# Antymon/ppo_cpp

Hardware: NVIDIA B200
Metric: ppo_env_steps_per_sec (higher is better)
Workload: dtype f32

## Files before the change

### ppo_cpp_b200/csrc/kernels_rollout.cuh

```cuda
#pragma once
#include <cooperative_groups.h>

#include "kernels_misc.cuh"
#include "kernels_mlp2.cuh"

namespace ppo {

struct RolloutArgs {
    NetDims d;
    const float* params;
    int n, T, tpc;
    uint64_t seed;
    uint32_t env_id0;
    uint32_t* step_ctr;
    SynthEnv env;
    NormStats st;
    float* ret;
    float norm_gamma, clip_obs, clip_rew, eps;
    int norm_obs, norm_reward, upd_obs, upd_ret;
    double* partial;
    float *cur_obs, *cur_dones, *last_values;
    float *obs_store, *act_store, *val_store, *nlp_store, *dones_store, *rew_store, *urew_store, *ret_store;
    float gamma, lam;
    unsigned *bar_ctr, *bar_gen;
    int n_global;
    PeerMailbox mbox;
    unsigned* mbox_seq;
    size_t off_obs, off_act, off_val, off_nlp, off_ret;
    size_t row_off;
    unsigned* done_seq;
    float* h_actions;
    size_t h_act_stride;
    const float *h_obs, *h_rew, *h_done;
    unsigned* h_act_flag;
    const unsigned* h_obs_flag;
    unsigned* host_err;
    int h_sentinel;
    uint2* h_act_ll;
    const uint2* h_ans_ll;
    long long* prof;
};

#define R_PROF()                                                                              \
    do {                                                                                      \
        if (a.prof && blockIdx.x == 0 && tid == 0 && t == 1 && prof_i < 32) a.prof[prof_i++] = clock64(); \
    } while (0)

constexpr int R_TM = 32, R_NTH = 256;
constexpr int R_SOLO_CHUNK = 32;
__host__ __device__ inline size_t rollout_solo_noise_bytes(int D) { return (size_t)2 * 2 * R_SOLO_CHUNK * 4 * ((D + 3) / 4) * sizeof(float) + 16; }
constexpr unsigned PPO_HOST_ENV_ABORT = 0xffffffffu;
constexpr unsigned PPO_OBS_SENTINEL = 0xffc0ffeeu;

__device__ __forceinline__ float* rslab(const RolloutArgs& a, int r, size_t off, int width, float* local) {
    return a.mbox.world > 1 ? reinterpret_cast<float*>(a.mbox.base[r] + off) + a.row_off * width : local;
}

struct RLayout {
    FLayout f;
    int obs, state, raw, ret, dn, tenv, res, rew, done, lastv, z2, mean, var, inv, misc, csum, total_bytes;
    __host__ __device__ void init(const NetDims& d, int tpc) {
        f.init(d, R_TM, false);
        int o = f.total;
        auto take = [&](int n) { int r = o; o += (n + 3) & ~3; return r; };
        obs = take(tpc * d.O * R_TM);
        state = take(tpc * d.O * R_TM);
        raw = take(tpc * d.O * R_TM);
        ret = take(tpc * R_TM); dn = take(tpc * R_TM); tenv = take(tpc * R_TM); res = take(tpc * R_TM);
        rew = take(tpc * R_TM); done = take(tpc * R_TM); lastv = take(tpc * R_TM);
        z2 = take(d.A * R_TM);
        mean = take(d.O + 1); var = take(d.O + 1); inv = take(d.O + 1); misc = take(8);
        o = (o + 1) & ~1;
        csum = o;
        o += 2 * (2 * (d.O + 1) + 2);
        total_bytes = o * 4;
    }
};

template <int O, int H1, int H2, int A, int TM>
__device__ __forceinline__ void solo_forward(const float* __restrict__ sW, const NetDims& d, const float* __restrict__ OBS, float* H1p, float* H1v,
                                             float* H2p, float* H2v, float* MU, float* Vs, int lane) {
#pragma unroll
    for (int i = 0; i < (2 * H1 + 31) / 32; ++i) {
        const int o = lane + 32 * i;
        if (o < 2 * H1) {
            const bool vt = o >= H1;
            const int n = vt ? o - H1 : o;
            const float* w = sW + d.off[vt ? T_VF_FC0_W : T_PI_FC0_W] + n;
            float acc = 0.f;
#pragma unroll
            for (int k = 0; k < O; ++k) acc = fmaf(w[k * H1], OBS[k * TM], acc);
            (vt ? H1v : H1p)[n * TM] = tanhf(acc + sW[d.off[vt ? T_VF_FC0_B : T_PI_FC0_B] + n]);
        }
    }
    __syncwarp();
#pragma unroll
    for (int i = 0; i < (2 * H2 + 31) / 32; ++i) {
        const int o = lane + 32 * i;
        if (o < 2 * H2) {
            const bool vt = o >= H2;
            const int n = vt ? o - H2 : o;
            const float* w = sW + d.off[vt ? T_VF_FC1_W : T_PI_FC1_W] + n;
            const float* hin = vt ? H1v : H1p;
            float acc = 0.f;
#pragma unroll
            for (int k = 0; k < H1; ++k) acc = fmaf(w[k * H2], hin[k * TM], acc);
            (vt ? H2v : H2p)[n * TM] = tanhf(acc + sW[d.off[vt ? T_VF_FC1_B : T_PI_FC1_B] + n]);
        }
    }
    __syncwarp();
    static_assert(A + 1 <= 32, "one lane per head output");
    if (lane < A + 1) {
        const bool vh = lane == A;
        const int N = vh ? 1 : A, n = vh ? 0 : lane;
        const float* w = sW + d.off[vh ? T_VF_W : T_PI_W] + n;
        const float* hin = vh ? H2v : H2p;
        float acc = 0.f;
#pragma unroll
        for (int k = 0; k < H2; ++k) acc = fmaf(w[k * N], hin[k * TM], acc);
        if (vh) Vs[0] = acc + sW[d.off[T_VF_B]];
        else MU[n * TM] = acc + sW[d.off[T_PI_B] + n];
    }
    __syncwarp();
}

__global__ void __launch_bounds__(R_NTH) rollout_persistent_kernel(const RolloutArgs a) {
    extern __shared__ __align__(16) float smem[];
    const NetDims& d = a.d;
    constexpr int TM = R_TM, NTH = R_NTH;
    const int O = d.O, A = d.A, D = d.O;
    RLayout L;
    L.init(d, a.tpc);
    float* sW = smem + L.f.w;
    float* Ac = smem + L.f.ac;
    float* MU = smem + L.f.mu;
    float* Vs = smem + L.f.vs;
    float* OBS = smem + L.obs;
    float* S = smem + L.state;
    float* RAW = smem + L.raw;
    float* RET = smem + L.ret;
    float* DN = smem + L.dn;
    uint32_t* TENV = reinterpret_cast<uint32_t*>(smem + L.tenv);
    uint32_t* RES = reinterpret_cast<uint32_t*>(smem + L.res);
    float* REW = smem + L.rew;
    float* DONE = smem + L.done;
    float* LASTV = smem + L.lastv;
    float* Z2 = smem + L.z2;
    float* s_mean = smem + L.mean;
    float* s_var = smem + L.var;
    float* s_inv = smem + L.inv;
    double* csum = reinterpret_cast<double*>(smem + L.csum);
    double* s_cnt = csum + 2 * (D + 1);

    const int tid = threadIdx.x, lane = tid & 31, warp = tid >> 5;
    constexpr int HALF = NTH / 2;
    const int tw = tid / HALF;
    const Sub half{tid % HALF, HALF};
    float* H1 = smem + L.f.h1[tw];
    float* H2 = smem + L.f.h2[tw];
    const int ntiles = (a.n + TM - 1) / TM;
    const int tile0 = blockIdx.x * a.tpc;
    const int my_tiles = max(0, min(a.tpc, ntiles - tile0));
    const int nblk = (D + 3) >> 2;
    const uint32_t step0 = *a.step_ctr;
    const bool merge = a.upd_obs || a.upd_ret;
    GridBarrier bar{a.bar_ctr, gridDim.x, *a.bar_gen};
    const int world = a.mbox.world;
    const bool host_env = a.h_actions != nullptr;
    __shared__ int s_abort;
    if (tid == 0) s_abort = 0;
    const unsigned seq0 = world > 1 ? *a.mbox_seq : 0u;
    const unsigned dseq0 = world > 1 ? *a.done_seq : 0u;

    stage_weights<NTH>(sW, a.params, d.P);
    if (tid < D) {
        s_mean[tid] = a.st.obs_mean[tid];
        s_var[tid] = a.st.obs_var[tid];
    } else if (tid == D) {
        s_mean[D] = *a.st.ret_mean;
        s_var[D] = *a.st.ret_var;
        s_cnt[0] = *a.st.obs_count;
        s_cnt[1] = *a.st.ret_count;
    }
    for (int tl = 0; tl < my_tiles; ++tl) {
        const int r0 = (tile0 + tl) * TM, nv = min(TM, a.n - r0);
        for (int e = tid; e < TM * D; e += NTH) {
            const int m = e / D, k = e - m * D;
            const bool ok = m < nv;
            OBS[(tl * O + k) * TM + m] = ok ? a.cur_obs[(size_t)(r0 + m) * O + k] : 0.f;
            S[(tl * TM + m) * D + k] = ok ? a.env.state[(size_t)(r0 + m) * D + k] : 0.f;
        }
        if (tid < TM) {
            const bool ok = tid < nv;
            RET[tl * TM + tid] = ok ? a.ret[r0 + tid] : 0.f;
            DN[tl * TM + tid] = ok ? a.cur_dones[r0 + tid] : 0.f;
            TENV[tl * TM + tid] = ok ? a.env.t_env[r0 + tid] : 0u;
            RES[tl * TM + tid] = ok ? a.env.resets[r0 + tid] : 0u;
        }
    }
    if (a.h_actions != nullptr && a.h_sentinel) {
        for (int tl = 0; tl < my_tiles; ++tl) {
            const int r0 = (tile0 + tl) * TM, nv = min(TM, a.n - r0);
            unsigned* dst = reinterpret_cast<unsigned*>(const_cast<float*>(a.h_obs) + (size_t)r0 * D);
            for (int i = tid; i < ((nv * D + 7) >> 3); i += NTH) dst[8 * i] = PPO_OBS_SENTINEL;
        }
    }
    cp_async_wait_all();
    bar.sync();

    const float* logstd = sW + d.off[T_LOGSTD];
    const uint2 ekey = make_uint2((uint32_t)a.env.seed, (uint32_t)(a.env.seed >> 32));

    int prof_i = 0;
    const bool solo_env = a.n == 1 && gridDim.x == 1 && world == 1;
    if (solo_env) {
        constexpr int CH = R_SOLO_CHUNK;
        const int NB = 4 * nblk;
        float* NZ = smem + ((L.total_bytes + 15) / 16) * 4;
        const uint32_t gid = a.env.env_id0;
        const uint32_t te0 = TENV[0];
        auto draw_chunk = [&](int c) {
            float* dst = NZ + (size_t)(c & 1) * 2 * CH * NB;
            const int per_kind = CH * nblk, total = host_env ? per_kind : 2 * per_kind;
            for (int e = tid - 32; e < total; e += NTH - 32) {
                const int kind = e / per_kind, r = e - kind * per_kind, s = r / nblk, blk = r - s * nblk, t = c * CH + s;
                if (t >= a.T) continue;
                float x4[4];
                if (kind == 0) normal4(a.seed, a.env_id0, step0 + (uint32_t)t, (uint32_t)blk, PPO_TAG_ACTION, x4);
                else normal4(a.env.seed, gid, te0 + (uint32_t)t, (uint32_t)blk, PPO_TAG_ENVNOISE, x4);
                float* o = dst + ((size_t)kind * CH + s) * NB + blk * 4;
                o[0] = x4[0]; o[1] = x4[1]; o[2] = x4[2]; o[3] = x4[3];
            }
        };
        if (warp > 0) draw_chunk(0);
        __syncthreads();
        float sl_c = 0.f;
        for (int j = 0; j < A; ++j) sl_c = __fadd_rn(sl_c, logstd[j]);
        const int nH1 = d.H1, nH2 = d.H2;
        const float *W0p = sW + d.off[T_PI_FC0_W], *W0v = sW + d.off[T_VF_FC0_W], *B0p = sW + d.off[T_PI_FC0_B], *B0v = sW + d.off[T_VF_FC0_B];
        const float *W1p = sW + d.off[T_PI_FC1_W], *W1v = sW + d.off[T_VF_FC1_W], *B1p = sW + d.off[T_PI_FC1_B], *B1v = sW + d.off[T_VF_FC1_B];
        const float *WHp = sW + d.off[T_PI_W], *WHv = sW + d.off[T_VF_W];
        float *H1p = smem + L.f.h1[0], *H1v = smem + L.f.h1[1], *H2p = smem + L.f.h2[0], *H2v = smem + L.f.h2[1];
        float sd_l[2];
        sd_l[0] = lane < A ? expf(logstd[lane]) : 1.f;
        sd_l[1] = lane + 32 < A ? expf(logstd[lane + 32]) : 1.f;
        for (int c = 0; c * CH < a.T; ++c) {
            if (warp > 0) {
                draw_chunk(c + 1);
            } else {
                const float* na = NZ + (size_t)(c & 1) * 2 * CH * NB;
                const float* ne = na + (size_t)CH * NB;
                for (int s = 0; s < CH && c * CH + s < a.T; ++s) {
                    const int t = c * CH + s;
                    R_PROF();
                    for (int k = lane; k < O; k += 32) a.obs_store[(size_t)t * O + k] = OBS[k * TM];
                    if (O == 18 && A == 18 && nH1 == 4 && nH2 == 5) {
                        solo_forward<18, 4, 5, 18, TM>(sW, d, OBS, H1p, H1v, H2p, H2v, MU, Vs, lane);
                    } else if (O == 18 && A == 18 && nH1 == 64 && nH2 == 64) {
                        solo_forward<18, 64, 64, 18, TM>(sW, d, OBS, H1p, H1v, H2p, H2v, MU, Vs, lane);
                    } else {
                    for (int o = lane; o < 2 * nH1; o += 32) {
                        const bool vt = o >= nH1;
                        const int n = vt ? o - nH1 : o;
                        const float* w = (vt ? W0v : W0p) + n;
                        float acc = 0.f;
#pragma unroll 6
                        for (int k = 0; k < O; ++k) acc = fmaf(w[k * nH1], OBS[k * TM], acc);
                        (vt ? H1v : H1p)[n * TM] = tanhf(acc + (vt ? B0v : B0p)[n]);
                    }
                    __syncwarp();
                    for (int o = lane; o < 2 * nH2; o += 32) {
                        const bool vt = o >= nH2;
                        const int n = vt ? o - nH2 : o;
                        const float* w = (vt ? W1v : W1p) + n;
                        const float* hin = vt ? H1v : H1p;
                        float acc = 0.f;
#pragma unroll 4
                        for (int k = 0; k < nH1; ++k) acc = fmaf(w[k * nH2], hin[k * TM], acc);
                        (vt ? H2v : H2p)[n * TM] = tanhf(acc + (vt ? B1v : B1p)[n]);
                    }
                    __syncwarp();
                    for (int o = lane; o < A + 1; o += 32) {
                        const bool vh = o == A;
                        const int N = vh ? 1 : A, n = vh ? 0 : o;
                        const float* w = (vh ? WHv : WHp) + n;
                        const float* hin = vh ? H2v : H2p;
                        float acc = 0.f;
#pragma unroll 4
                        for (int k = 0; k < nH2; ++k) acc = fmaf(w[k * N], hin[k * TM], acc);
                        if (vh) Vs[0] = acc + sW[d.off[T_VF_B]];
                        else MU[n * TM] = acc + sW[d.off[T_PI_B] + n];
                    }
                    __syncwarp();
                    }
                    R_PROF();
                    for (int j = lane, jj = 0; j < A; j += 32, ++jj) {
                        const float sd = jj ? sd_l[1] : sd_l[0];
                        const float mu = MU[j * TM];
                        const float act = __fadd_rn(mu, __fmul_rn(sd, na[s * NB + j]));
                        const float z = __fdiv_rn(__fsub_rn(act, mu), sd);
                        Ac[j * (TM + 1)] = act;
                        Z2[j * TM] = __fmul_rn(z, z);
                        a.act_store[(size_t)t * A + j] = act;
                        if (host_env) {
                            if (a.h_act_ll) ll_store(a.h_act_ll + j, __float_as_uint(act), (unsigned)t + 1u);
                            else a.h_actions[(size_t)t * a.h_act_stride + j] = act;
                        }
                    }
                    __syncwarp();
                    if (lane == 0) {
                        float ss = 0.f;
                        for (int j = 0; j < A; ++j) ss = __fadd_rn(ss, Z2[j * TM]);
                        a.nlp_store[t] = __fadd_rn(__fadd_rn(__fmul_rn(0.5f, ss), __fmul_rn(PPO_HALF_LOG_2PI, (float)A)), sl_c);
                        a.val_store[t] = Vs[0];
                        a.dones_store[t] = DN[0];
                    }
                    R_PROF();
                    if (host_env && a.h_ans_ll) {
                        const unsigned want = (unsigned)t + 1u;
                        uint2 w = make_uint2(0u, want);
                        bool gone = false;
                        if (lane < D + 2) {
                            const unsigned long long t0 = globaltimer_ns();
                            unsigned spins = 0;
                            while (true) {
                                w = ll_load(a.h_ans_ll + lane);
                                if (w.y == want) break;
                                if (w.y == PPO_HOST_ENV_ABORT) { gone = true; break; }
                                if (((++spins) & 0xffu) == 0u && globaltimer_ns() - t0 > 120000000000ull) {
                                    *a.host_err = 1u;
                                    gone = true;
                                    break;
                                }
                            }
                        }
                        if (__any_sync(0xffffffffu, gone)) {
                            if (lane == 0) s_abort = 1;
                            break;
                        }
                        if (lane < D) RAW[lane] = __uint_as_float(w.x);
                        else if (lane == D) REW[0] = __uint_as_float(w.x);
                        else if (lane == D + 1) DONE[0] = __uint_as_float(w.x);
                        __syncwarp();
                        if (lane == 0) RET[0] = __fadd_rn(__fmul_rn(RET[0], a.norm_gamma), REW[0]);
                    } else if (host_env) {
                        __syncwarp();
                        unsigned v = 0u;
                        if (lane == 0) {
                            __threadfence_system();
                            st_release_sys(a.h_act_flag, (unsigned)t + 1u);
                            const unsigned long long t0 = globaltimer_ns();
                            unsigned spins = 0;
                            while ((v = *reinterpret_cast<const volatile unsigned*>(a.h_obs_flag)) != (unsigned)t + 1u && v != PPO_HOST_ENV_ABORT) {
                                if (((++spins) & 0xffu) == 0u && globaltimer_ns() - t0 > 120000000000ull) {
                                    *a.host_err = 1u;
                                    v = PPO_HOST_ENV_ABORT;
                                    break;
                                }
                            }
                            __threadfence_system();
                        }
                        v = __shfl_sync(0xffffffffu, v, 0);
                        if (v == PPO_HOST_ENV_ABORT) {
                            if (lane == 0) s_abort = 1;
                            break;
                        }
                        for (int k = lane; k < D; k += 32) RAW[k] = __ldcv(a.h_obs + k);
                        if (lane == 0) {
                            REW[0] = __ldcv(a.h_rew);
                            DONE[0] = __ldcv(a.h_done);
                        }
                        __syncwarp();
                        if (lane == 0) RET[0] = __fadd_rn(__fmul_rn(RET[0], a.norm_gamma), REW[0]);
                    } else {
                        const uint32_t te = te0 + (uint32_t)t;
                        const bool dn = ((te + 1u) % 334u) == 0u;
                        for (int k = lane; k < D; k += 32) {
                            const float sk = S[k];
                            float ac = Ac[k * (TM + 1)];
                            ac = ac < -1.f ? -1.f : (ac > 1.f ? 1.f : ac);
                            float sn = __fadd_rn(__fadd_rn(__fmul_rn(0.9f, sk), __fmul_rn(0.1f, ac)), __fmul_rn(0.01f, ne[s * NB + k]));
                            if (k == 0) REW[0] = __fsub_rn(sn, sk);
                            if (dn) {
                                const uint4 w = philox4x32_10(make_uint4(gid, RES[0], (uint32_t)(k >> 2), PPO_TAG_ENVRESET), ekey);
                                const uint32_t wv[4] = {w.x, w.y, w.z, w.w};
                                sn = __fmul_rn(0.1f, __fsub_rn(__fmul_rn(2.0f, u32_to_unit(wv[k & 3])), 1.0f));
                            }
                            S[k] = sn;
                            RAW[k] = sn;
                        }
                        __syncwarp();
                        if (lane == 0) {
                            DONE[0] = dn ? 1.f : 0.f;
                            TENV[0] = te + 1u;
                            if (dn) RES[0] += 1u;
                            RET[0] = __fadd_rn(__fmul_rn(RET[0], a.norm_gamma), REW[0]);
                        }
                    }
                    __syncwarp();
                    R_PROF();
                    if (merge && lane <= D) {
                        const int cidx = lane;
                        const bool is_ret = cidx == D;
                        const double x = is_ret ? (double)RET[0] : (double)RAW[cidx] - (double)s_mean[cidx];
                        double ps = 0.0, pq = 0.0;
                        ps += x;
                        pq += x * x;
                        if (is_ret ? a.upd_ret : a.upd_obs) {
                            const double rows = (double)a.n_global;
                            const double pv = is_ret ? 0.0 : (double)s_mean[cidx];
                            const double m1 = ps;
                            const double mean_d = pv + m1;
                            double var_d = pq - m1 * m1;
                            if (var_d < 0.0) var_d = 0.0;
                            float mm = s_mean[cidx], vv = s_var[cidx];
                            chan_merge(mm, vv, s_cnt[is_ret ? 1 : 0], (float)mean_d, (float)var_d, rows);
                            s_mean[cidx] = mm;
                            s_var[cidx] = vv;
                        }
                    }
                    __syncwarp();
                    if (merge && lane == 0) {
                        if (a.upd_obs) s_cnt[0] = (double)a.n_global + s_cnt[0];
                        if (a.upd_ret) s_cnt[1] = (double)a.n_global + s_cnt[1];
                    }
                    R_PROF();
                    if (lane <= D) s_inv[lane] = __fdiv_rn(1.0f, __fsqrt_rn(__fadd_rn(s_var[lane], a.eps)));
                    __syncwarp();
                    for (int k = lane; k < D; k += 32) {
                        float x = RAW[k];
                        if (a.norm_obs) {
                            x = __fmul_rn(__fsub_rn(x, s_mean[k]), s_inv[k]);
                            x = fminf(fmaxf(x, -a.clip_obs), a.clip_obs);
                        }
                        OBS[k * TM] = x;
                    }
                    if (lane == 0) {
                        const float raw = REW[0];
                        float r = raw;
                        if (a.norm_reward) {
                            r = __fmul_rn(raw, s_inv[D]);
                            r = fminf(fmaxf(r, -a.clip_rew), a.clip_rew);
                        }
                        const float dn2 = DONE[0];
                        RET[0] = __fmul_rn(RET[0], __fsub_rn(1.0f, dn2));
                        DN[0] = dn2;
                        a.rew_store[t] = r;
                        a.urew_store[t] = raw;
                    }
                    __syncwarp();
                    R_PROF();
                }
            }
            __syncthreads();
            if (s_abort) break;
        }
    } else
    for (int t = 0; t < a.T; ++t) {
        const uint32_t step = step0 + (uint32_t)t;
        R_PROF();
        double ps = 0.0, pq = 0.0;
        const float pivot = (tid < D) ? s_mean[tid] : 0.f;
        for (int pass = 0; pass < (host_env ? 2 : 1); ++pass) {
        if (pass == 1) {
            __syncthreads();
            if (a.h_sentinel) {
                if (tid == 0) {
                    __threadfence_system();
                    st_release_sys(a.h_act_flag + blockIdx.x, (unsigned)t + 1u);
                }
                int gone = 0;
                const unsigned long long t0 = globaltimer_ns();
                for (int tl = 0; tl < my_tiles && !gone; ++tl) {
                    const int r0 = (tile0 + tl) * TM, nv = min(TM, a.n - r0);
                    const unsigned* src = reinterpret_cast<const unsigned*>(a.h_obs + (size_t)r0 * D);
                    const int nsec = (nv * D + 7) >> 3;
                    for (int i = tid; i < nsec && !gone; i += NTH) {
                        unsigned spins = 0;
                        while (__ldcv(src + 8 * i) == PPO_OBS_SENTINEL) {
                            if (((++spins) & 0x3fu) == 0u) {
                                if (__ldcv(a.h_obs_flag) == PPO_HOST_ENV_ABORT) { gone = 1; break; }
                                if (globaltimer_ns() - t0 > 120000000000ull) {
                                    *a.host_err = 1u;
                                    gone = 1;
                                    break;
                                }
                            }
                        }
                    }
                }
                const int any_gone = __syncthreads_or(gone);
                if (tid == 0) s_abort = any_gone;
                __syncthreads();
                if (s_abort) break;
            } else {
            if (tid == 0) {
                __threadfence_system();
                st_release_sys(a.h_act_flag + blockIdx.x, (unsigned)t + 1u);
                const unsigned long long t0 = globaltimer_ns();
                unsigned v, spins = 0;
                while ((v = *reinterpret_cast<const volatile unsigned*>(a.h_obs_flag)) != (unsigned)t + 1u && v != PPO_HOST_ENV_ABORT) {
                    if (((++spins) & 0xffu) == 0u && globaltimer_ns() - t0 > 120000000000ull) {
                        *a.host_err = 1u;
                        v = PPO_HOST_ENV_ABORT;
                        break;
                    }
                }
                s_abort = (v == PPO_HOST_ENV_ABORT) ? 1 : 0;
                __threadfence_system();
            }
            __syncthreads();
            if (s_abort) break;
            }
        }
        for (int tl = 0; tl < my_tiles; ++tl) {
            const int r0 = (tile0 + tl) * TM, nv = min(TM, a.n - r0);
            float* Xs = OBS + tl * O * TM;
            if (pass == 0) {
            for (int r = 0; r < world; ++r) {
                float* dst = rslab(a, r, a.off_obs, O, a.obs_store) + ((size_t)t * a.n + r0) * O;
                for (int e = tid; e < nv * O; e += NTH) {
                    const int m = e / O, k = e - m * O;
                    dst[e] = Xs[k * TM + m];
                }
            }
            f_fwd<TM, true>(Xs, O, sW + d.off[tw ? T_VF_FC0_W : T_PI_FC0_W], sW + d.off[tw ? T_VF_FC0_B : T_PI_FC0_B], d.H1, H1, half);
            __syncthreads();
            f_fwd<TM, true>(H1, d.H1, sW + d.off[tw ? T_VF_FC1_W : T_PI_FC1_W], sW + d.off[tw ? T_VF_FC1_B : T_PI_FC1_B], d.H2, H2, half);
            __syncthreads();
            if (tw == 0) f_fwd<TM, false>(H2, d.H2, sW + d.off[T_PI_W], sW + d.off[T_PI_B], A, MU, half);
            else f_fwd<TM, false>(H2, d.H2, sW + d.off[T_VF_W], sW + d.off[T_VF_B], 1, Vs, half);
            __syncthreads();
            R_PROF();
            for (int e = tid; e < TM * nblk; e += NTH) {
                const int m = e % TM, blk = e / TM;
                if (m < nv) {
                    float e4[4];
                    normal4(a.seed, a.env_id0 + (uint32_t)(r0 + m), step, (uint32_t)blk, PPO_TAG_ACTION, e4);
#pragma unroll
                    for (int q = 0; q < 4; ++q) {
                        const int j = blk * 4 + q;
                        if (j < A) {
                            const float sd = expf(logstd[j]);
                            const float mu = MU[j * TM + m];
                            const float act = __fadd_rn(mu, __fmul_rn(sd, e4[q]));
                            const float z = __fdiv_rn(__fsub_rn(act, mu), sd);
                            Ac[j * (TM + 1) + m] = act;
                            Z2[j * TM + m] = __fmul_rn(z, z);
                        }
                    }
                }
            }
            __syncthreads();
            if (tid < nv) {
                const int m = tid, row = r0 + m;
                float ss = 0.f, sl = 0.f;
                for (int j = 0; j < A; ++j) {
                    ss = __fadd_rn(ss, Z2[j * TM + m]);
                    sl = __fadd_rn(sl, logstd[j]);
                }
                const float nl = __fadd_rn(__fadd_rn(__fmul_rn(0.5f, ss), __fmul_rn(PPO_HALF_LOG_2PI, (float)A)), sl);
                const size_t idx = (size_t)t * a.n + row;
                for (int r = 0; r < world; ++r) {
                    rslab(a, r, a.off_nlp, 1, a.nlp_store)[idx] = nl;
                    rslab(a, r, a.off_val, 1, a.val_store)[idx] = Vs[m];
                }
                a.dones_store[idx] = DN[tl * TM + m];
            }
            for (int r = 0; r < world; ++r) {
                float* dst = rslab(a, r, a.off_act, A, a.act_store) + ((size_t)t * a.n + r0) * A;
                for (int e = tid; e < nv * A; e += NTH) {
                    const int m = e / A, j = e - m * A;
                    dst[e] = Ac[j * (TM + 1) + m];
                }
            }
            R_PROF();
            }
            if (host_env) {
                if (pass == 0) {
                    float* dst = a.h_actions + (size_t)t * a.h_act_stride + (size_t)r0 * A;
                    const int ne = nv * A;
                    if ((reinterpret_cast<uintptr_t>(dst) & 15) == 0) {
                        for (int e4 = tid; e4 < (ne >> 2); e4 += NTH) {
                            float v[4];
#pragma unroll
                            for (int i = 0; i < 4; ++i) {
                                const int e = 4 * e4 + i, m = e / A, j = e - m * A;
                                v[i] = Ac[j * (TM + 1) + m];
                            }
                            *reinterpret_cast<float4*>(dst + 4 * e4) = make_float4(v[0], v[1], v[2], v[3]);
                        }
                        for (int e = (ne & ~3) + tid; e < ne; e += NTH) {
                            const int m = e / A, j = e - m * A;
                            dst[e] = Ac[j * (TM + 1) + m];
                        }
                    } else {
                        for (int e = tid; e < ne; e += NTH) {
                            const int m = e / A, j = e - m * A;
                            dst[e] = Ac[j * (TM + 1) + m];
                        }
                    }
                    __syncthreads();
                    continue;
                }
                for (int e = tid; e < nv * D; e += NTH) RAW[tl * TM * D + e] = __ldcv(a.h_obs + (size_t)r0 * D + e);
                if (tid < nv) {
                    REW[tl * TM + tid] = __ldcv(a.h_rew + r0 + tid);
                    DONE[tl * TM + tid] = __ldcv(a.h_done + r0 + tid);
                }
                __syncthreads();
                if (a.h_sentinel) {
                    unsigned* dst = reinterpret_cast<unsigned*>(const_cast<float*>(a.h_obs) + (size_t)r0 * D);
                    for (int i = tid; i < ((nv * D + 7) >> 3); i += NTH) dst[8 * i] = PPO_OBS_SENTINEL;
                }
                if (tid < nv) RET[tl * TM + tid] = __fadd_rn(__fmul_rn(RET[tl * TM + tid], a.norm_gamma), REW[tl * TM + tid]);
                __syncthreads();
            } else {
            for (int e = tid; e < TM * nblk; e += NTH) {
                const int m = e % TM, blk = e / TM;
                if (m < nv) {
                    const uint32_t gid = a.env.env_id0 + (uint32_t)(r0 + m);
                    const uint32_t te = TENV[tl * TM + m];
                    const bool dn = ((te + 1u) % 334u) == 0u;
                    float xi[4];
                    normal4(a.env.seed, gid, te, (uint32_t)blk, PPO_TAG_ENVNOISE, xi);
                    float* st = S + (tl * TM + m) * D;
                    float* rw = RAW + (tl * TM + m) * D;
                    uint4 w = make_uint4(0, 0, 0, 0);
                    if (dn) w = philox4x32_10(make_uint4(gid, RES[tl * TM + m], (uint32_t)blk, PPO_TAG_ENVRESET), ekey);
                    const uint32_t wv[4] = {w.x, w.y, w.z, w.w};
#pragma unroll
                    for (int q = 0; q < 4; ++q) {
                        const int k = blk * 4 + q;
                        if (k < D) {
                            const float sk = st[k];
                            float ac = Ac[k * (TM + 1) + m];
                            ac = ac < -1.f ? -1.f : (ac > 1.f ? 1.f : ac);
                            float sn = __fadd_rn(__fadd_rn(__fmul_rn(0.9f, sk), __fmul_rn(0.1f, ac)), __fmul_rn(0.01f, xi[q]));
                            if (k == 0) REW[tl * TM + m] = __fsub_rn(sn, sk);
                            if (dn) sn = __fmul_rn(0.1f, __fsub_rn(__fmul_rn(2.0f, u32_to_unit(wv[q])), 1.0f));
                            st[k] = sn;
                            rw[k] = sn;
                        }
                    }
                    if (blk == 0) DONE[tl * TM + m] = dn ? 1.f : 0.f;
                }
            }
            __syncthreads();
            if (tid < nv) {
                const int m = tid;
                TENV[tl * TM + m] += 1u;
                if (DONE[tl * TM + m] != 0.f) RES[tl * TM + m] += 1u;
                RET[tl * TM + m] = __fadd_rn(__fmul_rn(RET[tl * TM + m], a.norm_gamma), REW[tl * TM + m]);
            }
            __syncthreads();
            }
            R_PROF();
            if (merge) {
                if (tid < D) {
                    for (int m = 0; m < nv; ++m) {
                        const double x = (double)RAW[(tl * TM + m) * D + tid] - (double)pivot;
                        ps += x;
                        pq += x * x;
                    }
                } else if (tid == D) {
                    for (int m = 0; m < nv; ++m) {
                        const double r = (double)RET[tl * TM + m];
                        ps += r;
                        pq += r * r;
                    }
                }
            }
        }
        }
        if (s_abort) break;
        if (merge) {
            const bool solo = gridDim.x == 1 && world == 1;
            double* mine = a.partial + (size_t)(t & 1) * 2 * (D + 1) * gridDim.x + blockIdx.x;
            if (solo) {
                if (tid <= D) {
                    csum[tid] = ps;
                    csum[D + 1 + tid] = pq;
                }
            } else if (tid <= D) {
                mine[(size_t)tid * gridDim.x] = ps;
                mine[(size_t)(D + 1 + tid) * gridDim.x] = pq;
            }
            R_PROF();
            if (!solo) bar.sync();
            R_PROF();
            const double* all = a.partial + (size_t)(t & 1) * 2 * (D + 1) * gridDim.x;
            if (!solo && (world == 1 || blockIdx.x == 0)) {
                constexpr int CPW = 5;
                double acc[CPW];
#pragma unroll
                for (int i = 0; i < CPW; ++i) acc[i] = 0.0;
#pragma unroll 4
                for (int b0 = 0; b0 < (int)gridDim.x; b0 += 32) {
                    double x[CPW];
#pragma unroll
                    for (int i = 0; i < CPW; ++i) {
                        const int c = warp + (NTH / 32) * i;
                        x[i] = (c < 2 * (D + 1) && b0 + lane < (int)gridDim.x) ? __ldcg(all + (size_t)c * gridDim.x + b0 + lane) : 0.0;
                    }
#pragma unroll
                    for (int i = 0; i < CPW; ++i) acc[i] += x[i];
                }
#pragma unroll
                for (int i = 0; i < CPW; ++i) {
                    const int c = warp + (NTH / 32) * i;
                    const double v = warp_sum(acc[i]);
                    if (lane == 0 && c < 2 * (D + 1)) csum[c] = v;
                }
                for (int c = (NTH / 32) * CPW + warp; c < 2 * (D + 1); c += NTH / 32) {
                    double v = 0.0;
                    for (int b = lane; b < (int)gridDim.x; b += 32) v += __ldcg(all + (size_t)c * gridDim.x + b);
                    v = warp_sum(v);
                    if (lane == 0) csum[c] = v;
                }
            }
            __syncthreads();
            if (world > 1) {
                const unsigned seq = seq0 + (unsigned)t + 1u;
                if (blockIdx.x == 0 && tid < 2 * (D + 1)) {
                    const unsigned long long bits = (unsigned long long)__double_as_longlong(csum[tid]);
                    for (int dst = 0; dst < world; ++dst) {
                        uint2* sl = a.mbox.ll_slot(dst, seq, a.mbox.rank) + 2 * tid;
                        ll_store(sl, (unsigned)bits, seq);
                        ll_store(sl + 1, (unsigned)(bits >> 32), seq);
                    }
                }
                __syncthreads();
                if (tid < 2 * (D + 1)) {
                    double v = 0.0;
                    for (int s0 = 0; s0 < world; s0 += 4) {
                        unsigned long long w[4];
                        a.mbox.ll_wait4_pair(seq, (size_t)(2 * tid), s0, w);
#pragma unroll
                        for (int k = 0; k < 4; ++k)
                            if (s0 + k < world) v += __longlong_as_double((long long)w[k]);
                    }
                    csum[tid] = v;
                }
                __syncthreads();
            }
            R_PROF();
            if (tid <= D) {
                const int c = tid;
                const bool is_ret = c == D;
                if (is_ret ? a.upd_ret : a.upd_obs) {
                    const double rows = (double)a.n_global;
                    const double pv = is_ret ? 0.0 : (double)s_mean[c];
                    const double m1 = csum[c] / rows;
                    const double mean_d = pv + m1;
                    double var_d = csum[D + 1 + c] / rows - m1 * m1;
                    if (var_d < 0.0) var_d = 0.0;
                    float mm = s_mean[c], vv = s_var[c];
                    chan_merge(mm, vv, s_cnt[is_ret ? 1 : 0], (float)mean_d, (float)var_d, rows);
                    s_mean[c] = mm;
                    s_var[c] = vv;
                }
            }
            __syncthreads();
            if (tid == 0) {
                if (a.upd_obs) s_cnt[0] = (double)a.n_global + s_cnt[0];
                if (a.upd_ret) s_cnt[1] = (double)a.n_global + s_cnt[1];
            }
        }
        R_PROF();
        if (tid <= D) s_inv[tid] = __fdiv_rn(1.0f, __fsqrt_rn(__fadd_rn(s_var[tid], a.eps)));
        __syncthreads();
        for (int tl = 0; tl < my_tiles; ++tl) {
            const int r0 = (tile0 + tl) * TM, nv = min(TM, a.n - r0);
            for (int e = tid; e < TM * D; e += NTH) {
                const int m = e / D, k = e - m * D;
                float x = RAW[(tl * TM + m) * D + k];
                if (a.norm_obs) {
                    x = __fmul_rn(__fsub_rn(x, s_mean[k]), s_inv[k]);
                    x = fminf(fmaxf(x, -a.clip_obs), a.clip_obs);
                }
                OBS[(tl * O + k) * TM + m] = (m < nv) ? x : 0.f;
            }
            if (tid < nv) {
                const int m = tid;
                const float raw = REW[tl * TM + m];
                float r = raw;
                if (a.norm_reward) {
                    r = __fmul_rn(raw, s_inv[D]);
                    r = fminf(fmaxf(r, -a.clip_rew), a.clip_rew);
                }
                const float dn = DONE[tl * TM + m];
                RET[tl * TM + m] = __fmul_rn(RET[tl * TM + m], __fsub_rn(1.0f, dn));
                DN[tl * TM + m] = dn;
                const size_t idx = (size_t)t * a.n + r0 + m;
                a.rew_store[idx] = r;
                a.urew_store[idx] = raw;
            }
        }
        __syncthreads();
        R_PROF();
    }

    for (int tl = 0; tl < my_tiles; ++tl) {
        const int r0 = (tile0 + tl) * TM, nv = min(TM, a.n - r0);
        float* Xs = OBS + tl * O * TM;
        if (tw == 1) f_fwd<TM, true>(Xs, O, sW + d.off[T_VF_FC0_W], sW + d.off[T_VF_FC0_B], d.H1, H1, half);
        __syncthreads();
        if (tw == 1) f_fwd<TM, true>(H1, d.H1, sW + d.off[T_VF_FC1_W], sW + d.off[T_VF_FC1_B], d.H2, H2, half);
        __syncthreads();
        if (tw == 1) f_fwd<TM, false>(H2, d.H2, sW + d.off[T_VF_W], sW + d.off[T_VF_B], 1, Vs, half);
        __syncthreads();
        if (tid < nv) LASTV[tl * TM + tid] = Vs[tid];
        for (int e = tid; e < nv * D; e += NTH) {
            const int m = e / D, k = e - m * D;
            a.cur_obs[(size_t)r0 * O + e] = Xs[k * TM + m];
            a.env.state[(size_t)r0 * D + e] = S[(tl * TM + m) * D + k];
        }
        __syncthreads();
    }
    for (int e = tid; e < my_tiles * TM; e += NTH) {
        const int tl = e / TM, m = e - tl * TM;
        const int row = (tile0 + tl) * TM + m;
        if (row >= a.n) continue;
        a.ret[row] = RET[e];
        a.cur_dones[row] = DN[e];
        a.env.t_env[row] = TENV[e];
        a.env.resets[row] = RES[e];
        a.last_values[row] = LASTV[e];
        const float gl = __fmul_rn(a.gamma, a.lam);
        float last = 0.f, nextv = LASTV[e], nextnt = 1.0f - DN[e];
#pragma unroll 8
        for (int t = a.T - 1; t >= 0; --t) {
            const size_t idx = (size_t)t * a.n + row;
            const float v = a.val_store[idx];
            const float delta = __fsub_rn(__fadd_rn(a.rew_store[idx], __fmul_rn(a.gamma, __fmul_rn(nextv, nextnt))), v);
            last = __fadd_rn(delta, __fmul_rn(gl, __fmul_rn(nextnt, last)));
            const float rt = __fadd_rn(last, v);
            for (int r = 0; r < world; ++r) rslab(a, r, a.off_ret, 1, a.ret_store)[idx] = rt;
            nextv = v;
            nextnt = 1.0f - a.dones_store[idx];
        }
    }
    if (world > 1) {
        __syncthreads();
        if (tid == 0) __threadfence_system();
        bar.sync();
        if (blockIdx.x == 0 && tid == 0) {
            a.mbox.signal_all(PPO_MBOX_DONE_CHANNEL, dseq0 + 1u);
            a.mbox.wait_all(PPO_MBOX_DONE_CHANNEL, dseq0 + 1u);
            *a.done_seq = dseq0 + 1u;
        }
    }
    if (blockIdx.x == 0) {
        if (tid < D) {
            a.st.obs_mean[tid] = s_mean[tid];
            a.st.obs_var[tid] = s_var[tid];
        } else if (tid == D) {
            *a.st.ret_mean = s_mean[D];
            *a.st.ret_var = s_var[D];
            *a.st.obs_count = s_cnt[0];
            *a.st.ret_count = s_cnt[1];
            *a.step_ctr = step0 + (uint32_t)a.T;
            *a.bar_gen = bar.gen;
            if (world > 1 && merge) *a.mbox_seq = seq0 + (unsigned)a.T;
        }
    }
}

}
```

Before: 36.93 million.

## Precompute action and env noise on idle threads during head layer

During the final head forward pass, threads not used by the policy/value head matmuls now generate the Philox normal noise for actions, environment noise and reset randoms, and store them in new shared-memory buffers. The later action-sampling and env-step loops read the precomputed noise instead of calling the RNG. The aim is to hide RNG latency inside an otherwise underused phase, at the cost of extra shared memory (which can lower occupancy) and a dependency on the idle-thread index arithmetic being correct. The profiling step index also changes.

After: 37.14 million (median of 6 runs). No clear change (+0.5%).

```diff
diff --git a/ppo_cpp_b200/csrc/kernels_rollout.cuh b/ppo_cpp_b200/csrc/kernels_rollout.cuh
--- a/ppo_cpp_b200/csrc/kernels_rollout.cuh
+++ b/ppo_cpp_b200/csrc/kernels_rollout.cuh
@@ -43,7 +43,7 @@
 
 #define R_PROF()                                                                              \
     do {                                                                                      \
-        if (a.prof && blockIdx.x == 0 && tid == 0 && t == 1 && prof_i < 32) a.prof[prof_i++] = clock64(); \
+        if (a.prof && blockIdx.x == 0 && tid == 0 && t == 8 && prof_i < 32) a.prof[prof_i++] = clock64(); \
     } while (0)
 
 constexpr int R_TM = 32, R_NTH = 256;
@@ -58,7 +58,7 @@
 
 struct RLayout {
     FLayout f;
-    int obs, state, raw, ret, dn, tenv, res, rew, done, lastv, z2, mean, var, inv, misc, csum, total_bytes;
+    int obs, state, raw, ret, dn, tenv, res, rew, done, lastv, z2, nza, nze, nzr, mean, var, inv, misc, csum, total_bytes;
     __host__ __device__ void init(const NetDims& d, int tpc) {
         f.init(d, R_TM, false);
         int o = f.total;
@@ -69,6 +69,8 @@
         ret = take(tpc * R_TM); dn = take(tpc * R_TM); tenv = take(tpc * R_TM); res = take(tpc * R_TM);
         rew = take(tpc * R_TM); done = take(tpc * R_TM); lastv = take(tpc * R_TM);
         z2 = take(d.A * R_TM);
+        const int nz = ((d.O + 3) / 4) * R_TM * 4;
+        nza = take(nz); nze = take(nz); nzr = take(nz);
         mean = take(d.O + 1); var = take(d.O + 1); inv = take(d.O + 1); misc = take(8);
         o = (o + 1) & ~1;
         csum = o;
@@ -146,6 +148,9 @@
     float* DONE = smem + L.done;
     float* LASTV = smem + L.lastv;
     float* Z2 = smem + L.z2;
+    float4* NZA = reinterpret_cast<float4*>(smem + L.nza);
+    float4* NZE = reinterpret_cast<float4*>(smem + L.nze);
+    uint4* NZR = reinterpret_cast<uint4*>(smem + L.nzr);
     float* s_mean = smem + L.mean;
     float* s_var = smem + L.var;
     float* s_inv = smem + L.inv;
@@ -530,13 +535,33 @@
             __syncthreads();
             if (tw == 0) f_fwd<TM, false>(H2, d.H2, sW + d.off[T_PI_W], sW + d.off[T_PI_B], A, MU, half);
             else f_fwd<TM, false>(H2, d.H2, sW + d.off[T_VF_W], sW + d.off[T_VF_B], 1, Vs, half);
+            {
+                const int hp = ((TM / 4) * ((A + 3) >> 2) + 31) & ~31, hv = ((TM / 4) + 31) & ~31;
+                const int idle = tw == 0 ? half.l - hp : (HALF - hp) + half.l - hv, nidle = 2 * HALF - hp - hv;
+                const int per = TM * nblk;
+                if (half.l >= (tw == 0 ? hp : hv))
+                    for (int e = idle; e < (host_env ? per : 2 * per); e += nidle) {
+                        const int kind = e >= per, r = e - kind * per, blk = r / TM, m = r - blk * TM;
+                        if (m >= nv) continue;
+                        float x4[4];
+                        if (kind == 0) {
+                            normal4(a.seed, a.env_id0 + (uint32_t)(r0 + m), step, (uint32_t)blk, PPO_TAG_ACTION, x4);
+                            NZA[r] = make_float4(x4[0], x4[1], x4[2], x4[3]);
+                        } else {
+                            const uint32_t gid = a.env.env_id0 + (uint32_t)(r0 + m), te = TENV[tl * TM + m];
+                            normal4(a.env.seed, gid, te, (uint32_t)blk, PPO_TAG_ENVNOISE, x4);
+                            NZE[r] = make_float4(x4[0], x4[1], x4[2], x4[3]);
+                            if (((te + 1u) % 334u) == 0u) NZR[r] = philox4x32_10(make_uint4(gid, RES[tl * TM + m], (uint32_t)blk, PPO_TAG_ENVRESET), ekey);
+                        }
+                    }
+            }
             __syncthreads();
             R_PROF();
             for (int e = tid; e < TM * nblk; e += NTH) {
                 const int m = e % TM, blk = e / TM;
                 if (m < nv) {
-                    float e4[4];
-                    normal4(a.seed, a.env_id0 + (uint32_t)(r0 + m), step, (uint32_t)blk, PPO_TAG_ACTION, e4);
+                    const float4 n4 = NZA[blk * TM + m];
+                    const float e4[4] = {n4.x, n4.y, n4.z, n4.w};
 #pragma unroll
                     for (int q = 0; q < 4; ++q) {
                         const int j = blk * 4 + q;
@@ -619,15 +644,14 @@
             for (int e = tid; e < TM * nblk; e += NTH) {
                 const int m = e % TM, blk = e / TM;
                 if (m < nv) {
-                    const uint32_t gid = a.env.env_id0 + (uint32_t)(r0 + m);
                     const uint32_t te = TENV[tl * TM + m];
                     const bool dn = ((te + 1u) % 334u) == 0u;
-                    float xi[4];
-                    normal4(a.env.seed, gid, te, (uint32_t)blk, PPO_TAG_ENVNOISE, xi);
+                    const float4 n4 = NZE[blk * TM + m];
+                    const float xi[4] = {n4.x, n4.y, n4.z, n4.w};
                     float* st = S + (tl * TM + m) * D;
                     float* rw = RAW + (tl * TM + m) * D;
                     uint4 w = make_uint4(0, 0, 0, 0);
-                    if (dn) w = philox4x32_10(make_uint4(gid, RES[tl * TM + m], (uint32_t)blk, PPO_TAG_ENVRESET), ekey);
+                    if (dn) w = NZR[blk * TM + m];
                     const uint32_t wv[4] = {w.x, w.y, w.z, w.w};
 #pragma unroll
                     for (int q = 0; q < 4; ++q) {
```
